# HeewoongNoh/DOSTransformer

Hardware: NVIDIA B200
Metric: train-step crystals/sec (fwd+bwd) (higher is better)
Workload: dtype bf16x3 operands, f32 accumulate

## Files before the change

### dostransformer_b200/_lib.py

```python
from __future__ import annotations

import ctypes as C
import os
from typing import Optional

import torch

_HERE = os.path.dirname(os.path.abspath(__file__))
LIB_PATH = os.environ.get("DOST_B200_LIB") or os.path.join(_HERE, "libdost_b200.so")

F32, F64 = 0, 1
ACT_NONE, ACT_RELU, ACT_LEAKY, ACT_PRELU = 0, 1, 2, 3
KC, MC = 0, 1
PREC_FMA, PREC_BF16X3, PREC_BF16 = 0, 1, 2
PRECISIONS = {"fp32": PREC_FMA, "bf16x3": PREC_BF16X3, "bf16": PREC_BF16}

_lib: Optional[C.CDLL] = None
ABI_VERSION = 15
DEVERR_MESSAGES = {1: "an index (edge_index / batch / system) is outside its table",
                   2: "a crystal has more atoms than the padding length given by the host (max_num_nodes)"}


class Seg(C.Structure):
    _fields_ = [("base", C.c_void_p), ("ld", C.c_longlong), ("idx", C.c_void_p), ("div", C.c_int),
# ... 36 lines not shown
        ("res_bstride", C.c_longlong),
        ("b_rowoff", C.c_void_p), ("c_rowoff", C.c_void_p), ("c_rowlim", C.c_void_p),
        ("colsum", C.c_void_p),
        ("out_gate", C.c_void_p), ("dact_gate", C.c_void_p), ("ld_gate", C.c_longlong),
    ]


_SIGNATURES = {
    "dost_abi_version": (C.c_int, []),
    "dost_last_error": (C.c_char_p, []),
    "dost_launch_count": (C.c_longlong, []),
    "dost_reset_launch_count": (None, []),
    "dost_device_errors_init": (C.c_int, []),
    "dost_device_errors": (C.c_uint, [C.c_int]),
    "dost_imax_scalar": (C.c_int, [C.c_void_p, C.c_int, C.c_void_p]),
    "dost_cast_i64_i32": (C.c_int, [C.c_void_p, C.c_void_p, C.c_longlong, C.c_void_p]),
    "dost_csr_workspace_bytes": (C.c_size_t, [C.c_longlong, C.c_longlong]),
    "dost_csr_build": (C.c_int, [C.c_void_p, C.c_longlong, C.c_longlong, C.c_void_p, C.c_void_p, C.c_void_p,
                                 C.c_void_p, C.c_size_t, C.c_void_p]),
    "dost_gemm_workspace_bytes": (C.c_size_t, [C.POINTER(Gemm)]),
    "dost_gemm": (C.c_int, [C.POINTER(Gemm), C.c_void_p, C.c_size_t, C.c_void_p]),
    "dost_gemm_bf16_workspace_bytes": (C.c_size_t, [C.POINTER(GemmBf16)]),
    "dost_gemm_bf16": (C.c_int, [C.POINTER(GemmBf16), C.c_void_p, C.c_size_t, C.c_void_p]),
    "dost_split_planes": (C.c_int, [C.c_void_p, C.c_longlong, C.c_longlong, C.c_int, C.c_void_p, C.c_void_p, C.c_longlong,
                                    C.c_void_p]),
    "dost_split_planes_multi": (C.c_int, [C.c_int, C.c_void_p, C.c_void_p, C.c_void_p, C.c_void_p, C.c_void_p, C.c_void_p,
                                          C.c_void_p, C.c_void_p]),
    "dost_split_planes_colsum_workspace_bytes": (C.c_size_t, [C.c_longlong, C.c_int, C.c_longlong]),
    "dost_split_planes_colsum": (C.c_int, [C.c_void_p, C.c_longlong, C.c_longlong, C.c_int, C.c_void_p, C.c_void_p, C.c_longlong,
                                           C.c_void_p, C.c_void_p, C.c_size_t, C.c_void_p]),
    "dost_ln_fwd_planes": (C.c_int, [C.c_void_p, C.c_longlong, C.c_void_p, C.c_void_p, C.c_void_p, C.c_void_p, C.c_longlong,
                                     C.c_void_p, C.c_void_p, C.c_void_p, C.c_void_p,
                                     C.c_void_p, C.c_void_p, C.c_longlong, C.c_void_p, C.c_longlong, C.c_int, C.c_void_p]),
    "dost_ln_bwd_planes_workspace_bytes": (C.c_size_t, [C.c_longlong, C.c_int]),
    "dost_ln_bwd_planes": (C.c_int, [C.c_void_p, C.c_longlong, C.c_void_p, C.c_longlong, C.c_void_p, C.c_void_p, C.c_void_p,
                                     C.c_void_p, C.c_void_p, C.c_longlong, C.c_void_p, C.c_void_p, C.c_void_p, C.c_longlong,
                                     C.c_void_p, C.c_void_p, C.c_void_p, C.c_void_p, C.c_longlong, C.c_int, C.c_void_p,
                                     C.c_size_t, C.c_void_p]),
    "dost_rowdot_fwd": (C.c_int, [C.c_void_p, C.c_longlong, C.c_void_p, C.c_void_p, C.c_void_p, C.c_longlong, C.c_int, C.c_void_p]),
    "dost_rowdot_bwd_workspace_bytes": (C.c_size_t, [C.c_longlong, C.c_int]),
    "dost_rowdot_bwd": (C.c_int, [C.c_void_p, C.c_void_p, C.c_longlong, C.c_void_p, C.c_void_p, C.c_void_p, C.c_longlong, C.c_int,
                                  C.c_void_p, C.c_size_t, C.c_void_p]),
    "dost_colsum_planes_workspace_bytes": (C.c_size_t, [C.c_longlong, C.c_int]),
    "dost_colsum_planes": (C.c_int, [C.c_void_p, C.c_void_p, C.c_longlong, C.c_longlong, C.c_int, C.c_void_p, C.c_void_p,
                                     C.c_size_t, C.c_void_p]),
    "dost_ln_fwd": (C.c_int, [C.c_int, C.c_void_p, C.c_longlong, C.c_void_p, C.c_void_p, C.c_void_p, C.c_void_p,
# ... 190 lines not shown
```

### dostransformer_b200/csrc/gemm_bf.cu

```cuda
#include <cuda.h>
#include <cuda_bf16.h>
#include <cstdlib>
#include "common.cuh"
#include "tc_ptx.cuh"

namespace dost {
namespace bf {

constexpr int BM = 128, BK = 64;
constexpr int kMaxStages = 6;
constexpr int kEpiBytes = 8 * 4096;
constexpr int kSmemBudget = 225 * 1024;

struct Maps {
  CUtensorMap a_hi[3], a_lo[3], b_hi, b_lo;
  CUtensorMap b_hi2, b_lo2;
  CUtensorMap c_out, c_hi, c_lo;
  CUtensorMap c_pre;
};

struct Params {
  int M, N, K;
  int a_nseg, a_kend[3];
  int a_mc, b_mc;
  int zmode, kchunk;
  long long c_bstride, res_bstride;
  const int* b_rowoff;
  const int* c_rowoff;
  const int* c_rowlim;
  int m_tiles, n_tiles, total_tiles;
  const float* bias;
  const float* rowbias; long long ld_rowbias; int rowbias_div;
  int act; float act_slope; const float* prelu_slope;
  float* out_pre; long long ld_pre;
  const __nv_bfloat16* dact_hi; long long ld_dact; float dact_slope;
  const float* residual; long long ld_res;
  float* out; long long ldc; int accumulate;
  __nv_bfloat16* out_hi; __nv_bfloat16* out_lo; long long ld_op;
  float* ws;
  float* colpart;
  unsigned int* out_gate;
  const unsigned int* dact_gate;
  long long ld_gate;
  int tma_epi;
};

// ... 115 lines not shown
                   : "memory");
      asm volatile("tcgen05.relinquish_alloc_permit.cta_group::1.sync.aligned;" ::: "memory");
    }
  }
  tc_fence_before();
  __syncthreads();
  if (CTA2) cluster_sync_all();
  tc_fence_after();
  const uint32_t tmem_base = tmem_base_s;
  const bool a_mc = p.a_mc != 0, b_mc = p.b_mc != 0;

  if (warp == kEpiWarps + 1) {
    if (lane == 0) {
      int stage = 0;
      uint32_t phase = 0;
      for (int tile = tile0; tile < p.total_tiles; tile += tile_step) {
        const TileInfo t = tile_info<BN, CTA2>(p, tile, rank);
        const int nb0 = t.n0 + rank * BNL;
        int seg = 0;
        for (int kt = 0; kt < t.nkt; ++kt) {
          const int k0 = t.kbeg + kt * BK;
          while (seg + 1 < p.a_nseg && k0 >= p.a_kend[seg]) ++seg;
          const int kseg = k0 - (seg == 0 ? 0 : p.a_kend[seg - 1]);
          mbar_wait(empty0 + 8 * stage, phase ^ 1);
          const uint32_t bar = CTA2 ? mapa_rank(full0 + 8 * stage, 0) : full0 + 8 * stage;
          if (!CTA2) mbar_expect_tx(bar, STAGE_BYTES);
          else if (rank == 0) mbar_expect_tx(full0 + 8 * stage, 2 * STAGE_BYTES);
          const uint32_t sA = smem_u32(smem + stage * STAGE_BYTES);
          const uint32_t sB = sA + (SPLIT ? 2 : 1) * A_BYTES;
          const int zb = (p.zmode == 1) ? t.z : 0;
          auto load = [&](uint32_t dst, const CUtensorMap* m, int c0, int c1, int c2) {
            if (CTA2) tma_load_3d_2cta(dst, m, c0, c1, c2, bar);
            else tma_load_3d(dst, m, c0, c1, c2, bar);
          };
          const int brow = p.b_rowoff ? __ldg(p.b_rowoff + t.z) : 0;
          const int zbb = p.b_rowoff ? 0 : zb;
          if (!a_mc) {
            load(sA, &maps.a_hi[seg], kseg, t.m0, zb);
            if (SPLIT) load(sA + A_BYTES, &maps.a_lo[seg], kseg, t.m0, zb);
          } else {
#pragma unroll
            for (int b = 0; b < BM / 64; ++b) {
              load(sA + b * 8192, &maps.a_hi[0], t.m0 + 64 * b, k0, zb);
              if (SPLIT) load(sA + A_BYTES + b * 8192, &maps.a_lo[0], t.m0 + 64 * b, k0, zb);
            }
          }
          if (!b_mc) {
            load(sB, CTA2 ? &maps.b_hi2 : &maps.b_hi, k0, nb0 + brow, zbb);
            if (SPLIT) load(sB + B_BYTES, CTA2 ? &maps.b_lo2 : &maps.b_lo, k0, nb0 + brow, zbb);
          } else {
#pragma unroll
            for (int b = 0; b < BNL / 64; ++b) {
              load(sB + b * 8192, &maps.b_hi, nb0 + 64 * b, k0 + brow, zbb);
              if (SPLIT) load(sB + B_BYTES + b * 8192, &maps.b_lo, nb0 + 64 * b, k0 + brow, zbb);
            }
          }
          if (++stage == NSTAGE) {
            stage = 0;
            phase ^= 1;
          }
        }
      }
    }
  } else if (warp == kEpiWarps) {
    const uint32_t idesc = make_idesc(CTA2 ? 2 * BM : BM, BN, a_mc, b_mc);
    const uint32_t a_kstep = a_mc ? (2048 >> 4) : (32 >> 4);
    const uint32_t b_kstep = b_mc ? (2048 >> 4) : (32 >> 4);
    int stage = 0;
    uint32_t phase = 0;
    uint32_t acc_phase[2] = {0, 0};
    int local = 0;
    for (int tile = tile0; tile < p.total_tiles && rank == 0; tile += tile_step, ++local) {
      const TileInfo t = tile_info<BN, CTA2>(p, tile, rank);
      const int buf = local & 1;
      mbar_wait(acce0 + 8 * buf, acc_phase[buf] ^ 1);
      tc_fence_after();
      const uint32_t tmem_d = tmem_base + buf * BN;
// ... 746 lines not shown
  attr[0].val.clusterDim.x = 2;
  attr[0].val.clusterDim.y = 1;
  attr[0].val.clusterDim.z = 1;
  cfg.attrs = attr;
  cfg.numAttrs = 1;
  cudaError_t e = cudaLaunchKernelEx(&cfg, kern, maps, p);
  if (e != cudaSuccess) {
    set_error("gemm_bf16: cluster launch failed: %s", cudaGetErrorString(e));
    return DOST_ERR_LAUNCH;
  }
  return check_launch("gemm_bf16 (CTA pairs)");
}

static bool use_cta_pairs(int M, int N) {
  static const int enabled = [] {
    const char* e = getenv("DOST_GEMM_2CTA");
    return (e && e[0] == '0') ? 0 : 1;
  }();
  return enabled && M > 128 && N > 128;
}

static inline bool al16(const void* ptr) { return (reinterpret_cast<uintptr_t>(ptr) & 15) == 0; }

static int run(const dost_gemm_bf16_t* h, void* workspace, size_t workspace_bytes, cudaStream_t st) {
  DOST_REQUIRE(h->M > 0 && h->N > 0 && h->K > 0, "gemm_bf16: bad shape M=%d N=%d K=%d", h->M, h->N, h->K);
  DOST_REQUIRE(h->precision == DOST_PREC_BF16X3 || h->precision == DOST_PREC_BF16, "gemm_bf16: precision must be bf16x3 or bf16");
  DOST_REQUIRE(h->N % 4 == 0, "gemm_bf16: N must be a multiple of 4 (got %d)", h->N);
  const bool split3 = h->precision == DOST_PREC_BF16X3;
  const bool a_mc = h->a_mode == DOST_MC, b_mc = h->b_mode == DOST_MC;
  const int nseg = a_mc ? 1 : h->a_nseg;
  DOST_REQUIRE(nseg >= 1 && nseg <= 3, "gemm_bf16: a_nseg must be 1..3");
  const int bn = h->N <= 64 ? 64 : (h->N <= 128 ? 128 : 256);
  const bool pairs = use_cta_pairs(h->M, h->N);
  const int batch = h->batch < 1 ? 1 : h->batch;
  DOST_REQUIRE(!(batch > 1 && h->split_k > 1), "gemm_bf16: batch and split_k are exclusive");
  DOST_REQUIRE(batch == 1 || (h->a_nseg <= 1 && !h->rowbias && !h->out_pre && !h->dact_hi && !h->out_hi),
               "gemm_bf16: batched problems support bias / activation / residual / fp32 stores only");
  DOST_REQUIRE(batch == 1 || (h->a_bstride % 8 == 0 && h->b_bstride % 8 == 0 && h->c_bstride % 4 == 0 && h->res_bstride % 4 == 0),
               "gemm_bf16: batch strides must keep 16-byte alignment");

  Maps maps;
  Params p;
  p.M = h->M; p.N = h->N; p.K = h->K;
  p.a_nseg = nseg;
  p.a_mc = a_mc; p.b_mc = b_mc;
  int kacc = 0;
  for (int s = 0; s < nseg; ++s) {
    const dost_planes_t& pl = h->a[s];
    DOST_REQUIRE(pl.hi && (!split3 || pl.lo), "gemm_bf16: A segment %d planes missing", s);
    DOST_REQUIRE(al16(pl.hi) && al16(pl.lo) && pl.ld % 8 == 0, "gemm_bf16: A segment %d planes must be 16-byte aligned, ld %% 8 == 0", s);
    const int width = a_mc ? h->K : pl.width;
    if (nseg > 1) DOST_REQUIRE(width % BK == 0, "gemm_bf16: concatenated A segments need widths %% 64 == 0 (got %d)", width);
    kacc += width;
    p.a_kend[s] = kacc;
    int rc;
    if (!a_mc) {
      const long long rows = batch > 1 ? h->M : pl.rows;
      rc = make_map(&maps.a_hi[s], pl.hi, width, rows, pl.ld, BM, batch, h->a_bstride);
      if (rc == DOST_OK && split3) rc = make_map(&maps.a_lo[s], pl.lo, width, rows, pl.ld, BM, batch, h->a_bstride);
    } else {
      rc = make_map(&maps.a_hi[s], pl.hi, h->M, h->K, pl.ld, 64, batch, h->a_bstride);
      if (rc == DOST_OK && split3) rc = make_map(&maps.a_lo[s], pl.lo, h->M, h->K, pl.ld, 64, batch, h->a_bstride);
    }
    if (rc != DOST_OK) return rc;
    if (!split3) maps.a_lo[s] = maps.a_hi[s];
  }
  for (int s = nseg; s < 3; ++s) {
    maps.a_hi[s] = maps.a_hi[0];
    maps.a_lo[s] = maps.a_lo[0];
    p.a_kend[s] = kacc;
  }
  DOST_REQUIRE(kacc == h->K, "gemm_bf16: A segment widths sum to %d, K=%d", kacc, h->K);
  {
    const dost_planes_t& pl = h->b;
    DOST_REQUIRE(pl.hi && (!split3 || pl.lo), "gemm_bf16: B planes missing");
    DOST_REQUIRE(al16(pl.hi) && al16(pl.lo) && pl.ld % 8 == 0, "gemm_bf16: B planes must be 16-byte aligned, ld %% 8 == 0");
    int rc;
    const bool ragged_b = h->b_rowoff != nullptr;
    if (ragged_b) {
      DOST_REQUIRE(pl.rows > 0, "gemm_bf16: ragged B needs the total number of stored rows");
      if (!b_mc) {
        rc = make_map(&maps.b_hi, pl.hi, h->K, pl.rows, pl.ld, bn);
        if (rc == DOST_OK && split3) rc = make_map(&maps.b_lo, pl.lo, h->K, pl.rows, pl.ld, bn);
        if (rc == DOST_OK && pairs) rc = make_map(&maps.b_hi2, pl.hi, h->K, pl.rows, pl.ld, 128);
        if (rc == DOST_OK && pairs && split3) rc = make_map(&maps.b_lo2, pl.lo, h->K, pl.rows, pl.ld, 128);
      } else {
        rc = make_map(&maps.b_hi, pl.hi, h->N, pl.rows, pl.ld, 64);
        if (rc == DOST_OK && split3) rc = make_map(&maps.b_lo, pl.lo, h->N, pl.rows, pl.ld, 64);
      }
    } else if (!b_mc) {
      const long long nrows = (pl.rows > 0 && pl.rows < h->N) ? pl.rows : h->N;
      rc = make_map(&maps.b_hi, pl.hi, h->K, nrows, pl.ld, bn, batch, h->b_bstride);
      if (rc == DOST_OK && split3) rc = make_map(&maps.b_lo, pl.lo, h->K, nrows, pl.ld, bn, batch, h->b_bstride);
      if (rc == DOST_OK && pairs) rc = make_map(&maps.b_hi2, pl.hi, h->K, nrows, pl.ld, 128, batch, h->b_bstride);
      if (rc == DOST_OK && pairs && split3) rc = make_map(&maps.b_lo2, pl.lo, h->K, nrows, pl.ld, 128, batch, h->b_bstride);
    } else {
      rc = make_map(&maps.b_hi, pl.hi, h->N, h->K, pl.ld, 64, batch, h->b_bstride);
      if (rc == DOST_OK && split3) rc = make_map(&maps.b_lo, pl.lo, h->N, h->K, pl.ld, 64, batch, h->b_bstride);
    }
    if (rc != DOST_OK) return rc;
    if (!split3) maps.b_lo = maps.b_hi;
    if (!pairs || b_mc) maps.b_hi2 = maps.b_hi;
    if (!pairs || b_mc || !split3) maps.b_lo2 = maps.b_hi2;
  }
  const int split = h->split_k < 1 ? 1 : h->split_k;
  p.zmode = split > 1 ? 2 : (batch > 1 ? 1 : 0);
  p.c_bstride = h->c_bstride;
  p.res_bstride = h->res_bstride;
  p.b_rowoff = h->b_rowoff;
  p.c_rowoff = h->c_rowoff;
  p.c_rowlim = h->c_rowlim;
  DOST_REQUIRE(!p.c_rowoff || p.c_rowlim, "gemm_bf16: ragged output needs both c_rowoff and c_rowlim");
  DOST_REQUIRE(split == 1 || !(p.b_rowoff || p.c_rowoff || p.c_rowlim), "gemm_bf16: ragged problems cannot be split along K");
  p.kchunk = 0;
  p.ws = nullptr;
  if (split > 1) {
    DOST_REQUIRE(!h->bias && !h->rowbias && h->act == DOST_ACT_NONE && !h->out_pre && !h->dact_hi && !h->residual && !h->out_hi,
                 "gemm_bf16: split_k supports only plain (accumulating) fp32 stores");
    const size_t need = sizeof(float) * (size_t)split * h->M * h->N;
    if (!workspace || workspace_bytes < need) {
      set_error("gemm_bf16: split_k workspace too small (%zu < %zu)", workspace_bytes, need);
      return DOST_ERR_WORKSPACE;
    }
    int kchunk = (h->K + split - 1) / split;
    p.kchunk = ((kchunk + BK - 1) / BK) * BK;
    p.ws = (float*)workspace;
// ... 21 lines not shown
  p.colpart = nullptr;
  const int nrb = (h->M + 31) / 32;
  if (h->colsum) {
    DOST_REQUIRE(split == 1 && batch == 1, "gemm_bf16: colsum needs a plain (single, un-split) problem");
    const size_t need = sizeof(float) * ((size_t)nrb + kMidRows) * h->N;
    if (!workspace || workspace_bytes < need) {
      set_error("gemm_bf16: colsum workspace too small (%zu < %zu)", workspace_bytes, need);
      return DOST_ERR_WORKSPACE;
    }
    p.colpart = (float*)workspace;
  }
  DOST_REQUIRE(h->out || h->out_hi, "gemm_bf16: no output");
  DOST_REQUIRE(!h->out || (al16(h->out) && h->ldc % 4 == 0), "gemm_bf16: out must be 16-byte aligned with ldc %% 4 == 0");
  DOST_REQUIRE(!h->bias || al16(h->bias), "gemm_bf16: bias must be 16-byte aligned");
  DOST_REQUIRE(!h->rowbias || (al16(h->rowbias) && h->ld_rowbias % 4 == 0), "gemm_bf16: rowbias alignment");
  DOST_REQUIRE(!h->out_pre || (al16(h->out_pre) && h->ld_pre % 4 == 0), "gemm_bf16: out_pre alignment");
  DOST_REQUIRE(!h->residual || (al16(h->residual) && h->ld_res % 4 == 0), "gemm_bf16: residual alignment");
  DOST_REQUIRE(!h->dact_hi || (((uintptr_t)h->dact_hi & 7) == 0 && h->ld_dact % 4 == 0), "gemm_bf16: dact plane alignment");
  DOST_REQUIRE(!h->out_hi || (((uintptr_t)h->out_hi & 7) == 0 && ((uintptr_t)h->out_lo & 7) == 0 && h->ld_op % 4 == 0),
               "gemm_bf16: output plane alignment");

  p.tma_epi = 0;
  bool ew16 = false;
  maps.c_out = maps.b_hi;
  maps.c_hi = maps.b_hi;
  maps.c_lo = maps.b_hi;
  maps.c_pre = maps.b_hi;
  if (tma_epi_enabled() && split == 1 && !(h->accumulate && h->out_hi) && !p.c_rowoff && !p.c_rowlim &&
      !(h->out_pre && !h->out) && (batch == 1 || !h->out_hi) && h->M >= 32 && h->N >= 32 && !(h->dact_hi && h->residual) &&
      (!h->dact_hi || (al16(h->dact_hi) && h->ld_dact % 8 == 0))) {
    int rc2 = DOST_OK;
    ew16 = pairs && epi16_enabled(h->colsum != nullptr);
    const int bc = ew16 ? 16 : 32;
    if (h->out) rc2 = make_out_map(&maps.c_out, h->out, true, bc, h->N, h->M, h->ldc, batch, h->c_bstride);
    if (rc2 == DOST_OK && h->out_pre) rc2 = make_out_map(&maps.c_pre, h->out_pre, true, bc, h->N, h->M, h->ld_pre);
    if (rc2 == DOST_OK && h->out_hi) {
      if (al16(h->out_hi) && al16(h->out_lo) && h->ld_op % 8 == 0) {
        rc2 = make_out_map(&maps.c_hi, h->out_hi, false, bc, h->N, h->M, h->ld_op);
        if (rc2 == DOST_OK && h->out_lo) rc2 = make_out_map(&maps.c_lo, h->out_lo, false, bc, h->N, h->M, h->ld_op);
      } else {
        rc2 = DOST_ERR_ARG;
      }
    }
    if (rc2 == DOST_OK) p.tma_epi = 1;
    else ew16 = false;
  }

  if ((h->out_gate || h->dact_gate) && !p.tma_epi) {
    set_error("gemm_bf16: activation gates are implemented by the TMA-store epilogue only (this launch is not eligible)");
    return DOST_ERR_UNSUPPORTED;
// ... 17 lines not shown
  }
  if (split > 1) {
    const long long total4 = (long long)h->M * h->N / 4;
    int blocks = (int)min64((total4 + 255) / 256, (long long)kNumSMs * 8);
    if (blocks < 1) blocks = 1;
    splitk_reduce_kernel<<<blocks, 256, 0, st>>>(p.ws, h->out, h->ldc, h->M, h->N, split, h->accumulate);
    rc = check_launch("gemm_bf16 split-k reduce");
  }
  return rc;
}

}
}

extern "C" size_t dost_gemm_bf16_workspace_bytes(const dost_gemm_bf16_t* g) {
  if (!g) return 0;
  if (g->colsum) return sizeof(float) * ((size_t)((g->M + 31) / 32) + dost::bf::kMidRows) * g->N;
  if (g->split_k <= 1) return 0;
  return sizeof(float) * (size_t)g->split_k * g->M * g->N;
}

extern "C" int dost_gemm_bf16(const dost_gemm_bf16_t* g, void* workspace, size_t workspace_bytes, dost_stream_t stream) {
  DOST_REQUIRE(g != nullptr, "gemm_bf16: null descriptor");
  return dost::bf::run(g, workspace, workspace_bytes, (cudaStream_t)stream);
}

extern "C" size_t dost_split_planes_colsum_workspace_bytes(long long rows, int cols, long long ldp) {
  return sizeof(float) * (size_t)dost::bf::split_colsum_chunks(rows, (int)ldp) * cols;
}

extern "C" int dost_split_planes_colsum(const float* x, long long ld, long long rows, int cols, void* hi, void* lo, long long ldp,
                                        float* colsum, void* workspace, size_t workspace_bytes, dost_stream_t stream) {
  DOST_REQUIRE(x && hi && colsum, "split_planes_colsum: null pointer");
  DOST_REQUIRE(rows > 0 && cols > 0 && ldp >= cols && ldp % 8 == 0, "split_planes_colsum: need rows > 0, ldp %% 8 == 0, ldp >= cols");
  DOST_REQUIRE(((uintptr_t)hi & 15) == 0 && ((uintptr_t)lo & 15) == 0, "split_planes_colsum: planes must be 16-byte aligned");
  const int nch = dost::bf::split_colsum_chunks(rows, (int)ldp);
  const size_t need = sizeof(float) * (size_t)nch * cols;
  if (!workspace || workspace_bytes < need) {
    dost::set_error("split_planes_colsum: workspace too small (%zu < %zu)", workspace_bytes, need);
    return DOST_ERR_WORKSPACE;
  }
  const int vec_ok = (((uintptr_t)x & 15) == 0 && ld % 4 == 0) ? 1 : 0;
  const long long rpc = (rows + nch - 1) / nch;
  dim3 grid((unsigned)((ldp / 8 + 31) / 32), nch);
  cudaStream_t st = (cudaStream_t)stream;
  dost::bf::split_planes_colsum_kernel<<<grid, 256, 0, st>>>(x, ld, rows, cols, (__nv_bfloat16*)hi, (__nv_bfloat16*)lo, (int)ldp, vec_ok,
                                                             rpc, (float*)workspace);
// ... 55 lines not shown
```

### dostransformer_b200/ops.py

```python
from __future__ import annotations

import ctypes as C
import math
from contextlib import nullcontext
import os
from dataclasses import dataclass, field
from typing import List, Optional, Sequence, Tuple

import torch

from . import _lib as L

NUM_SMS = 148

_PRECISION = L.PREC_FMA


def set_precision(name: str) -> None:
    global _PRECISION
    _PRECISION = L.PRECISIONS[name]


def get_precision() -> int:
    return _PRECISION
# ... 361 lines not shown
        cache[_planes_key(w)] = ((base._version, base.data_ptr(), _PLANES_GENERATION), Planes(hi, lo, w.shape[0], w.shape[1]))


def _planes_c(pl: Planes, width: int) -> L.PlanesC:
    c = L.PlanesC()
    c.hi = pl.hi.data_ptr()
    c.lo = pl.lo.data_ptr() if pl.lo is not None else None
    c.ld = pl.ld
    c.rows = pl.rows
    c.width = width
    return c


def gemm_planes(*, M: int, N: int, K: int, a: Sequence[Planes], a_mode: int, b: Planes, b_mode: int,
                out: Optional[torch.Tensor] = None, bias: Optional[torch.Tensor] = None,
                rowbias: Optional[torch.Tensor] = None, rowbias_div: int = 1, act: int = L.ACT_NONE, act_slope: float = 0.0,
                prelu_slope: Optional[torch.Tensor] = None, out_pre: Optional[torch.Tensor] = None,
                dact: Optional[Planes] = None, dact_slope: float = 0.0, residual: Optional[torch.Tensor] = None,
                accumulate: bool = False, split_k: int = 1, out_planes: Optional[Planes] = None,
                ldc: Optional[int] = None, prec: Optional[int] = None, batch: int = 1, a_bstride: int = 0, b_bstride: int = 0,
                c_bstride: int = 0, res_bstride: int = 0, ld_res: Optional[int] = None, b_rows: Optional[int] = None,
                b_rowoff: Optional[torch.Tensor] = None, c_rowoff: Optional[torch.Tensor] = None,
                c_rowlim: Optional[torch.Tensor] = None, colsum_out: Optional[torch.Tensor] = None,
                out_gate: Optional[torch.Tensor] = None, dact_gate: Optional[torch.Tensor] = None) -> None:
    g = L.GemmBf16()
    g.M, g.N, g.K = M, N, K
    g.a_mode, g.a_nseg = a_mode, len(a)
    for i, pl in enumerate(a):
        g.a[i] = _planes_c(pl, pl.cols if a_mode == L.KC else K)
    g.b_mode = b_mode
    g.b = _planes_c(b, 0)
    g.b.rows = b_rows if b_rows is not None else 0
    g.bias = bias.data_ptr() if bias is not None else None
    if rowbias is not None:
        g.rowbias, g.ld_rowbias, g.rowbias_div = rowbias.data_ptr(), _ld(rowbias), rowbias_div
    g.act, g.act_slope = act, act_slope
    g.prelu_slope = prelu_slope.data_ptr() if prelu_slope is not None else None
    if out_pre is not None:
        g.out_pre, g.ld_pre = out_pre.data_ptr(), _ld(out_pre)
    if dact is not None:
        g.dact_hi, g.ld_dact, g.dact_slope = dact.hi.data_ptr(), dact.ld, dact_slope
    if residual is not None:
        g.residual, g.ld_res = residual.data_ptr(), (ld_res if ld_res is not None else _ld(residual))
    if out is not None:
        g.out = out.data_ptr()
        g.ldc = ldc if ldc is not None else _ld(out)
    g.accumulate = 1 if accumulate else 0
    g.batch, g.a_bstride, g.b_bstride, g.c_bstride, g.res_bstride = batch, a_bstride, b_bstride, c_bstride, res_bstride
    g.b_rowoff = b_rowoff.data_ptr() if b_rowoff is not None else None
    g.c_rowoff = c_rowoff.data_ptr() if c_rowoff is not None else None
    g.c_rowlim = c_rowlim.data_ptr() if c_rowlim is not None else None
    if out_planes is not None:
        g.out_hi = out_planes.hi.data_ptr()
        g.out_lo = out_planes.lo.data_ptr() if out_planes.lo is not None else None
        g.ld_op = out_planes.ld
    g.split_k = split_k
    g.precision = _PRECISION if prec is None else prec
    g.colsum = colsum_out.data_ptr() if colsum_out is not None else None
    if out_gate is not None:
        g.out_gate, g.ld_gate = out_gate.data_ptr(), out_gate.stride(0)
    if dact_gate is not None:
        g.dact_gate, g.ld_gate, g.dact_slope = dact_gate.data_ptr(), dact_gate.stride(0), dact_slope
    lib = L.lib()
    ws, nb = None, 0
    if split_k > 1 or colsum_out is not None:
        nb = lib.dost_gemm_bf16_workspace_bytes(C.byref(g))
        ws = _ws(nb, b.hi.device)
    L.check(lib.dost_gemm_bf16(C.byref(g), L.p(ws), nb, L.stream()), "gemm_bf16")


def gate_bits_ok(M: int, N: int) -> bool:
    return M >= 32 and N % 32 == 0 and os.environ.get("DOST_GEMM_TMA_EPI", "1") != "0" and not L.switch("DOST_NO_FFN_GATE")


def tc_active(t: torch.Tensor) -> bool:
    return _PRECISION != L.PREC_FMA and t.dtype == torch.float32


def _with_lo() -> bool:
    return _PRECISION != L.PREC_BF16


def ln_fwd_planes(x2d: torch.Tensor, gamma, beta, slope=None, *, want_y: bool = False, want_planes: bool = True,
                  gather_add=None):
    M, W = x2d.shape
    ga = ia = gb = ib = None
    ldg = 0
    if gather_add is not None:
        ga, ia, gb, ib = gather_add
        ldg = _ld(ga)
        assert _ld(gb) == ldg
# ... 869 lines not shown
            dop = _grad_planes(d_out, S * T, H)
            d_out = d_out.contiguous()
            dP = torch.empty(S * T, npad, dtype=torch.float32, device=dev)
            gemm_planes(M=T, N=npad, K=H, a=[dop], a_mode=L.KC, b=kvp, b_mode=L.KC, b_rows=N + B, out=dP, batch=S,
                        a_bstride=T * dop.ld, c_bstride=T * npad, b_rowoff=ptr_ext)
            dsp = empty_planes(S * T, npad, dev, _with_lo())
            if ctx.fused and ctx.drop_p > 0:
                scores = torch.empty(S * T, npad, dtype=torch.float32, device=dev)
                gemm_planes(M=T, N=npad, K=H, a=[qp], a_mode=L.KC, b=kvp, b_mode=L.KC, b_rows=N + B, out=scores, batch=S,
                            a_bstride=T * qp.ld, c_bstride=T * npad, b_rowoff=ptr_ext)
            if ctx.fused and ctx.drop_p == 0:
                _ds_from_planes(pp, dP, S * T, npad, float(H) ** -0.5, dsp)
            else:
                L.check(lib.dost_xattn_softmax_bwd_dseed(L.p(scores), L.p(lse), L.p(dP), L.p(g.ptr), L.p(g.nmax), S * T, B, T, npad,
                                                         float(H) ** -0.5, L.p(dsp.hi), L.p(dsp.lo), dsp.ld, ctx.drop_p, ctx.seed,
                                                         L.p(ctx.seed_offset), L.stream()), "xattn_softmax_bwd")
            dq = torch.empty(S, T, H, dtype=torch.float32, device=dev)
            gemm_planes(M=T, N=H, K=npad, a=[dsp], a_mode=L.KC, b=kvp, b_mode=L.MC, b_rows=N + B, out=dq.view(S * T, H), batch=S,
                        a_bstride=T * dsp.ld, c_bstride=T * H, b_rowoff=ptr_ext)
            dkv = torch.empty(N, H, dtype=torch.float32, device=dev)
            dbrows = torch.empty(B, H, dtype=torch.float32, device=dev)
            if not L.switch("DOST_NO_XATTN_PADDED_DK"):
                dpad = torch.empty(S * npad, H, dtype=torch.float32, device=dev)
                gemm_planes(M=npad, N=H, K=T, a=[dsp], a_mode=L.MC, b=qp, b_mode=L.MC, out=dpad, batch=S, a_bstride=T * dsp.ld,
                            b_bstride=T * qp.ld, c_bstride=npad * H)
                gemm_planes(M=npad, N=H, K=T, a=[pp], a_mode=L.MC, b=dop, b_mode=L.MC, out=dpad, accumulate=True, batch=S,
                            a_bstride=T * pp.ld, b_bstride=T * dop.ld, c_bstride=npad * H)
                L.check(lib.dost_xattn_kv_pad_split(L.p(dpad), npad, reps, L.p(g.batch), L.p(g.ptr), N, B, H, L.p(dkv), L.p(dbrows),
                                                    L.stream()), "xattn_kv_pad_split")
                dph = colsum(dbrows)
                d_q = colsum(dq.view(S, T * H)).view(T, H) if ctx.bcast_q else dq
                d_resid = colsum(d_out.view(S, T * H)).view(T, H) if ctx.bcast_r else d_out
                return d_q, dkv, dph, d_resid, None, None, None, None, None, None
            dext = torch.empty(N + B, H, dtype=torch.float32, device=dev)
            p1, n1 = g.ragged(1)
            for rep in range(reps):
                r0, r1 = rep * B * T, (rep + 1) * B * T
                gemm_planes(M=npad, N=H, K=T, a=[_rows(dsp, r0, r1)], a_mode=L.MC, b=_rows(qp, r0, r1), b_mode=L.MC, out=dext,
                            accumulate=rep > 0, batch=B, a_bstride=T * dsp.ld, b_bstride=T * qp.ld, c_rowoff=p1, c_rowlim=n1)
                gemm_planes(M=npad, N=H, K=T, a=[_rows(pp, r0, r1)], a_mode=L.MC, b=_rows(dop, r0, r1), b_mode=L.MC, out=dext,
                            accumulate=True, batch=B, a_bstride=T * pp.ld, b_bstride=T * dop.ld, c_rowoff=p1, c_rowlim=n1)
            L.check(lib.dost_xattn_kv_ext_split(L.p(dext), L.p(g.batch), L.p(g.ptr), N, B, H, L.p(dkv), L.p(dbrows), L.stream()),
                    "xattn_kv_ext_split")
            dph = colsum(dbrows)
            d_q = colsum(dq.view(S, T * H)).view(T, H) if ctx.bcast_q else dq
            d_resid = colsum(d_out.view(S, T * H)).view(T, H) if ctx.bcast_r else d_out
        return d_q, dkv, dph, d_resid, None, None, None, None, None, None


def _rows(pl: Planes, r0: int, r1: int) -> Planes:
# ... 108 lines not shown
    qp, kp = Planes(qh, ql, S * Lq, H), Planes(kh, kl, S * Lk, H)
    pdp = Planes(ph, pl_, S * Lq, Lk)
    dop = _grad_planes(d_out, S * Lq, H)
    d_out = d_out.contiguous()
    dpd = torch.empty(S, Lq, Lp, dtype=torch.float32, device=dev)
    gemm_planes(M=Lq, N=Lp, K=H, a=[dop], a_mode=L.KC, b=kp, b_mode=L.KC, b_rows=Lk, out=dpd.view(S * Lq, Lp), batch=S,
                a_bstride=Lq * dop.ld, b_bstride=Lk * kp.ld, c_bstride=Lq * Lp)
    dsp = empty_planes(S * Lq, Lk, dev, _with_lo())
    if ctx.fused and ctx.drop_p > 0:
        prob = torch.empty(S, Lq, Lp, dtype=torch.float32, device=dev)
        gemm_planes(M=Lq, N=Lp, K=H, a=[qp], a_mode=L.KC, b=kp, b_mode=L.KC, b_rows=Lk, out=prob.view(S * Lq, Lp), batch=S,
                    a_bstride=Lq * qp.ld, b_bstride=Lk * kp.ld, c_bstride=Lq * Lp)
        L.check(L.lib().dost_softmax_fwd(L.F32, L.p(prob), L.p(prob), None, S * Lq, Lk, Lp, scale, 0.0, 0, L.stream()), "softmax_fwd")
    if ctx.fused and ctx.drop_p == 0:
        _ds_from_planes(pdp, dpd.view(S * Lq, Lp), S * Lq, Lk, scale, dsp)
    else:
        L.check(L.lib().dost_softmax_bwd_planes_dseed(L.p(prob), L.p(dpd), None, S * Lq, Lk, Lp, scale, ctx.drop_p, ctx.seed,
                                                      L.p(ctx.seed_offset), L.p(dsp.hi), L.p(dsp.lo), dsp.ld, L.stream()),
                "softmax_bwd_planes")
    dq = torch.empty(S, Lq, H, dtype=torch.float32, device=dev)
    gemm_planes(M=Lq, N=H, K=Lk, a=[dsp], a_mode=L.KC, b=kp, b_mode=L.MC, out=dq.view(S * Lq, H), batch=S,
                a_bstride=Lq * dsp.ld, b_bstride=Lk * kp.ld, c_bstride=Lq * H)
    dk = torch.empty(S, Lk, H, dtype=torch.float32, device=dev)
    gemm_planes(M=Lk, N=H, K=Lq, a=[dsp], a_mode=L.MC, b=qp, b_mode=L.MC, out=dk.view(S * Lk, H), batch=S,
                a_bstride=Lq * dsp.ld, b_bstride=Lq * qp.ld, c_bstride=Lk * H)
    gemm_planes(M=Lk, N=H, K=Lq, a=[pdp], a_mode=L.MC, b=dop, b_mode=L.MC, out=dk.view(S * Lk, H), accumulate=True, batch=S,
                a_bstride=Lq * pdp.ld, b_bstride=Lq * dop.ld, c_bstride=Lk * H)
    return dq, dk, d_out, None, None, None


_SelfAttention._backward_planes = staticmethod(_self_attention_backward_planes)


def _cols(pl: Planes, cols: int) -> Planes:
    return Planes(pl.hi, pl.lo, pl.rows, cols)


def _planes3(t: torch.Tensor) -> Optional[Planes]:
    pl = getattr(t, "_dost_planes", None)
    if pl is not None and t.dim() == 3 and pl.rows == t.shape[0] * t.shape[1] and pl.cols == t.shape[2] and \
            (pl.lo is not None) == _with_lo():
        return pl
    return None


def self_attention(q, k, resid, drop_p: float = 0.0, seed: int = 0, seed_offset=None):
    _check_seed_offset(seed_offset)
    out = _SelfAttention.apply(q, k, resid, drop_p, seed, seed_offset)
    if tc_active(q) and q.shape[-1] % 8 == 0:
        out._dost_attn_out = True
# ... 91 lines not shown
```

### include/dost.h

```cpp
#ifndef DOST_H_
#define DOST_H_

#include <stddef.h>
#include <stdint.h>

#ifdef __cplusplus
extern "C" {
#endif

#define DOST_ABI_VERSION 15

enum { DOST_F32 = 0, DOST_F64 = 1 };
enum { DOST_OK = 0, DOST_ERR_ARG = -1, DOST_ERR_LAUNCH = -2, DOST_ERR_WORKSPACE = -3, DOST_ERR_UNSUPPORTED = -4 };
enum { DOST_ACT_NONE = 0, DOST_ACT_RELU = 1, DOST_ACT_LEAKY = 2, DOST_ACT_PRELU = 3 };
enum { DOST_PREC_FMA = 0, DOST_PREC_BF16X3 = 1 , DOST_PREC_BF16 = 2 };
enum { DOST_KC = 0 , DOST_MC = 1  };

typedef void* dost_stream_t;

int dost_abi_version(void);
const char* dost_last_error(void);
long long dost_launch_count(void);
void dost_reset_launch_count(void);

// ... 60 lines not shown
  const float* bias;
  const float* rowbias; long long ld_rowbias; int rowbias_div;
  int act; float act_slope; const float* prelu_slope;
  float* out_pre; long long ld_pre;
  const void* dact_hi; long long ld_dact; float dact_slope;
  const float* residual; long long ld_res;
  float* out; long long ldc; int accumulate;
  void* out_hi; void* out_lo; long long ld_op;
  int split_k;
  int precision;
  int batch;
  long long a_bstride, b_bstride, c_bstride, res_bstride;
  const int32_t* b_rowoff;
  const int32_t* c_rowoff;
  const int32_t* c_rowlim;
  float* colsum;
  uint32_t* out_gate;
  const uint32_t* dact_gate;
  long long ld_gate;
} dost_gemm_bf16_t;

size_t dost_gemm_bf16_workspace_bytes(const dost_gemm_bf16_t* g);
int dost_gemm_bf16(const dost_gemm_bf16_t* g, void* workspace, size_t workspace_bytes, dost_stream_t stream);
int dost_split_planes_multi(int ntensors, const float* const* x, const long long* ld, const long long* rows, const int* cols,
                            void* const* hi, void* const* lo, const long long* ldp, dost_stream_t stream);
int dost_split_planes(const float* x, long long ld, long long rows, int cols, void* hi, void* lo, long long ldp,
                      dost_stream_t stream);
size_t dost_split_planes_colsum_workspace_bytes(long long rows, int cols, long long ldp);
int dost_split_planes_colsum(const float* x, long long ld, long long rows, int cols, void* hi, void* lo, long long ldp,
                             float* colsum, void* workspace, size_t workspace_bytes, dost_stream_t stream);

int dost_ln_fwd_planes(float* x, long long ldx, const float* ga, const int32_t* ia, const float* gb, const int32_t* ib,
                       long long ldg, const float* gamma, const float* beta, const float* prelu_slope, float* y,
                       void* hi, void* lo, long long ldp, float* stats, long long M, int W, dost_stream_t stream);
size_t dost_ln_bwd_planes_workspace_bytes(long long M, int W);
int dost_ln_bwd_planes(const float* dy, long long ld_dy, const float* x, long long ldx, const float* stats,
                       const float* gamma, const float* beta, const float* prelu_slope, const float* dres,
                       long long ld_dres, float* dx, void* dx_hi, void* dx_lo, long long ldp, float* dgamma,
                       float* dbeta, float* dslope, float* dxsum, long long M, int W, void* workspace,
                       size_t workspace_bytes, dost_stream_t stream);
int dost_rowdot_fwd(const float* x, long long ldx, const float* w, const float* bias, float* out, long long M, int K,
                    dost_stream_t stream);
size_t dost_rowdot_bwd_workspace_bytes(long long M, int K);
int dost_rowdot_bwd(const float* dout, const float* x, long long ldx, const float* w, float* dx, float* dwb, long long M, int K,
                    void* workspace, size_t workspace_bytes, dost_stream_t stream);
size_t dost_colsum_planes_workspace_bytes(long long M, int W);
// ... 146 lines not shown
```

Baseline: 21360.

## Fuse two accumulating attention-backward GEMMs into one two-product GEMM launch

```diff
diff --git a/dostransformer_b200/_lib.py b/dostransformer_b200/_lib.py
--- a/dostransformer_b200/_lib.py
+++ b/dostransformer_b200/_lib.py
@@ -82,6 +82,7 @@
     "dost_gemm": (C.c_int, [C.POINTER(Gemm), C.c_void_p, C.c_size_t, C.c_void_p]),
     "dost_gemm_bf16_workspace_bytes": (C.c_size_t, [C.POINTER(GemmBf16)]),
     "dost_gemm_bf16": (C.c_int, [C.POINTER(GemmBf16), C.c_void_p, C.c_size_t, C.c_void_p]),
+    "dost_gemm_bf16_two_products": (C.c_int, [C.POINTER(GemmBf16), C.POINTER(PlanesC), C.c_void_p, C.c_size_t, C.c_void_p]),
     "dost_split_planes": (C.c_int, [C.c_void_p, C.c_longlong, C.c_longlong, C.c_int, C.c_void_p, C.c_void_p, C.c_longlong,
                                     C.c_void_p]),
     "dost_split_planes_multi": (C.c_int, [C.c_int, C.c_void_p, C.c_void_p, C.c_void_p, C.c_void_p, C.c_void_p, C.c_void_p,
diff --git a/dostransformer_b200/csrc/gemm_bf.cu b/dostransformer_b200/csrc/gemm_bf.cu
--- a/dostransformer_b200/csrc/gemm_bf.cu
+++ b/dostransformer_b200/csrc/gemm_bf.cu
@@ -13,8 +13,9 @@
 constexpr int kSmemBudget = 225 * 1024;
 
 struct Maps {
-  CUtensorMap a_hi[3], a_lo[3], b_hi, b_lo;
-  CUtensorMap b_hi2, b_lo2;
+  CUtensorMap a_hi[3], a_lo[3];
+  CUtensorMap b_hi[2], b_lo[2];
+  CUtensorMap b_hi2[2], b_lo2[2];
   CUtensorMap c_out, c_hi, c_lo;
   CUtensorMap c_pre;
 };
@@ -22,6 +23,7 @@
 struct Params {
   int M, N, K;
   int a_nseg, a_kend[3];
+  int b_seg;
   int a_mc, b_mc;
   int zmode, kchunk;
   long long c_bstride, res_bstride;
@@ -183,6 +185,8 @@
           const int k0 = t.kbeg + kt * BK;
           while (seg + 1 < p.a_nseg && k0 >= p.a_kend[seg]) ++seg;
           const int kseg = k0 - (seg == 0 ? 0 : p.a_kend[seg - 1]);
+          const int bs = p.b_seg ? seg : 0;
+          const int kb = p.b_seg ? kseg : k0;
           mbar_wait(empty0 + 8 * stage, phase ^ 1);
           const uint32_t bar = CTA2 ? mapa_rank(full0 + 8 * stage, 0) : full0 + 8 * stage;
           if (!CTA2) mbar_expect_tx(bar, STAGE_BYTES);
@@ -202,18 +206,18 @@
           } else {
 #pragma unroll
             for (int b = 0; b < BM / 64; ++b) {
-              load(sA + b * 8192, &maps.a_hi[0], t.m0 + 64 * b, k0, zb);
-              if (SPLIT) load(sA + A_BYTES + b * 8192, &maps.a_lo[0], t.m0 + 64 * b, k0, zb);
+              load(sA + b * 8192, &maps.a_hi[seg], t.m0 + 64 * b, kseg, zb);
+              if (SPLIT) load(sA + A_BYTES + b * 8192, &maps.a_lo[seg], t.m0 + 64 * b, kseg, zb);
             }
           }
           if (!b_mc) {
-            load(sB, CTA2 ? &maps.b_hi2 : &maps.b_hi, k0, nb0 + brow, zbb);
-            if (SPLIT) load(sB + B_BYTES, CTA2 ? &maps.b_lo2 : &maps.b_lo, k0, nb0 + brow, zbb);
+            load(sB, CTA2 ? &maps.b_hi2[bs] : &maps.b_hi[bs], kb, nb0 + brow, zbb);
+            if (SPLIT) load(sB + B_BYTES, CTA2 ? &maps.b_lo2[bs] : &maps.b_lo[bs], kb, nb0 + brow, zbb);
           } else {
 #pragma unroll
             for (int b = 0; b < BNL / 64; ++b) {
-              load(sB + b * 8192, &maps.b_hi, nb0 + 64 * b, k0 + brow, zbb);
-              if (SPLIT) load(sB + B_BYTES + b * 8192, &maps.b_lo, nb0 + 64 * b, k0 + brow, zbb);
+              load(sB + b * 8192, &maps.b_hi[bs], nb0 + 64 * b, kb + brow, zbb);
+              if (SPLIT) load(sB + B_BYTES + b * 8192, &maps.b_lo[bs], nb0 + 64 * b, kb + brow, zbb);
             }
           }
           if (++stage == NSTAGE) {
@@ -1006,20 +1010,28 @@
 
 static inline bool al16(const void* ptr) { return (reinterpret_cast<uintptr_t>(ptr) & 15) == 0; }
 
-static int run(const dost_gemm_bf16_t* h, void* workspace, size_t workspace_bytes, cudaStream_t st) {
+static int run(const dost_gemm_bf16_t* h, const dost_planes_t* b_seg1, void* workspace, size_t workspace_bytes, cudaStream_t st) {
   DOST_REQUIRE(h->M > 0 && h->N > 0 && h->K > 0, "gemm_bf16: bad shape M=%d N=%d K=%d", h->M, h->N, h->K);
   DOST_REQUIRE(h->precision == DOST_PREC_BF16X3 || h->precision == DOST_PREC_BF16, "gemm_bf16: precision must be bf16x3 or bf16");
   DOST_REQUIRE(h->N % 4 == 0, "gemm_bf16: N must be a multiple of 4 (got %d)", h->N);
   const bool split3 = h->precision == DOST_PREC_BF16X3;
   const bool a_mc = h->a_mode == DOST_MC, b_mc = h->b_mode == DOST_MC;
-  const int nseg = a_mc ? 1 : h->a_nseg;
+  const bool bseg = b_seg1 != nullptr;
+  const int nseg = (a_mc && !bseg) ? 1 : h->a_nseg;
   DOST_REQUIRE(nseg >= 1 && nseg <= 3, "gemm_bf16: a_nseg must be 1..3");
+  DOST_REQUIRE(!bseg || nseg == 2, "gemm_bf16: a second B needs a_nseg == 2");
   const int bn = h->N <= 64 ? 64 : (h->N <= 128 ? 128 : 256);
   const bool pairs = use_cta_pairs(h->M, h->N);
   const int batch = h->batch < 1 ? 1 : h->batch;
   DOST_REQUIRE(!(batch > 1 && h->split_k > 1), "gemm_bf16: batch and split_k are exclusive");
-  DOST_REQUIRE(batch == 1 || (h->a_nseg <= 1 && !h->rowbias && !h->out_pre && !h->dact_hi && !h->out_hi),
-               "gemm_bf16: batched problems support bias / activation / residual / fp32 stores only");
+  DOST_REQUIRE(batch == 1 || ((h->a_nseg <= 1 || bseg) && !h->rowbias && !h->out_pre && !h->dact_hi && !h->out_hi),
+               "gemm_bf16: batched problems support bias / activation / residual / fp32 stores / two products only");
+  DOST_REQUIRE(!bseg || batch == 1 || (h->a[1].ld == h->a[0].ld && b_seg1->ld == h->b.ld),
+               "gemm_bf16: batched two-product problems need equal plane pitches of both pairs");
+  if (bseg && (h->split_k > 1 || h->b_rowoff)) {
+    set_error("gemm_bf16: two-product problems cannot be split along K or use a ragged B");
+    return DOST_ERR_UNSUPPORTED;
+  }
   DOST_REQUIRE(batch == 1 || (h->a_bstride % 8 == 0 && h->b_bstride % 8 == 0 && h->c_bstride % 4 == 0 && h->res_bstride % 4 == 0),
                "gemm_bf16: batch strides must keep 16-byte alignment");
 
@@ -1027,15 +1039,18 @@
   Params p;
   p.M = h->M; p.N = h->N; p.K = h->K;
   p.a_nseg = nseg;
+  p.b_seg = bseg ? 1 : 0;
   p.a_mc = a_mc; p.b_mc = b_mc;
-  int kacc = 0;
+  int kacc = 0, ksum = 0;
   for (int s = 0; s < nseg; ++s) {
     const dost_planes_t& pl = h->a[s];
     DOST_REQUIRE(pl.hi && (!split3 || pl.lo), "gemm_bf16: A segment %d planes missing", s);
     DOST_REQUIRE(al16(pl.hi) && al16(pl.lo) && pl.ld % 8 == 0, "gemm_bf16: A segment %d planes must be 16-byte aligned, ld %% 8 == 0", s);
-    const int width = a_mc ? h->K : pl.width;
-    if (nseg > 1) DOST_REQUIRE(width % BK == 0, "gemm_bf16: concatenated A segments need widths %% 64 == 0 (got %d)", width);
-    kacc += width;
+    const int width = (a_mc && !bseg) ? h->K : pl.width;
+    DOST_REQUIRE(width > 0, "gemm_bf16: A segment %d is empty", s);
+    if (nseg > 1 && !bseg) DOST_REQUIRE(width % BK == 0, "gemm_bf16: concatenated A segments need widths %% 64 == 0 (got %d)", width);
+    ksum += width;
+    kacc += (bseg && s + 1 < nseg) ? (width + BK - 1) / BK * BK : width;
     p.a_kend[s] = kacc;
     int rc;
     if (!a_mc) {
@@ -1043,8 +1058,8 @@
       rc = make_map(&maps.a_hi[s], pl.hi, width, rows, pl.ld, BM, batch, h->a_bstride);
       if (rc == DOST_OK && split3) rc = make_map(&maps.a_lo[s], pl.lo, width, rows, pl.ld, BM, batch, h->a_bstride);
     } else {
-      rc = make_map(&maps.a_hi[s], pl.hi, h->M, h->K, pl.ld, 64, batch, h->a_bstride);
-      if (rc == DOST_OK && split3) rc = make_map(&maps.a_lo[s], pl.lo, h->M, h->K, pl.ld, 64, batch, h->a_bstride);
+      rc = make_map(&maps.a_hi[s], pl.hi, h->M, width, pl.ld, 64, batch, h->a_bstride);
+      if (rc == DOST_OK && split3) rc = make_map(&maps.a_lo[s], pl.lo, h->M, width, pl.ld, 64, batch, h->a_bstride);
     }
     if (rc != DOST_OK) return rc;
     if (!split3) maps.a_lo[s] = maps.a_hi[s];
@@ -1054,9 +1069,11 @@
     maps.a_lo[s] = maps.a_lo[0];
     p.a_kend[s] = kacc;
   }
-  DOST_REQUIRE(kacc == h->K, "gemm_bf16: A segment widths sum to %d, K=%d", kacc, h->K);
-  {
-    const dost_planes_t& pl = h->b;
+  DOST_REQUIRE(ksum == h->K, "gemm_bf16: A segment widths sum to %d, K=%d", ksum, h->K);
+  p.K = kacc;
+  for (int s = 0; s < (bseg ? 2 : 1); ++s) {
+    const dost_planes_t& pl = s == 0 ? h->b : *b_seg1;
+    const int kb = bseg ? h->a[s].width : h->K;
     DOST_REQUIRE(pl.hi && (!split3 || pl.lo), "gemm_bf16: B planes missing");
     DOST_REQUIRE(al16(pl.hi) && al16(pl.lo) && pl.ld % 8 == 0, "gemm_bf16: B planes must be 16-byte aligned, ld %% 8 == 0");
     int rc;
@@ -1064,28 +1081,32 @@
     if (ragged_b) {
       DOST_REQUIRE(pl.rows > 0, "gemm_bf16: ragged B needs the total number of stored rows");
       if (!b_mc) {
-        rc = make_map(&maps.b_hi, pl.hi, h->K, pl.rows, pl.ld, bn);
-        if (rc == DOST_OK && split3) rc = make_map(&maps.b_lo, pl.lo, h->K, pl.rows, pl.ld, bn);
-        if (rc == DOST_OK && pairs) rc = make_map(&maps.b_hi2, pl.hi, h->K, pl.rows, pl.ld, 128);
-        if (rc == DOST_OK && pairs && split3) rc = make_map(&maps.b_lo2, pl.lo, h->K, pl.rows, pl.ld, 128);
+        rc = make_map(&maps.b_hi[s], pl.hi, kb, pl.rows, pl.ld, bn);
+        if (rc == DOST_OK && split3) rc = make_map(&maps.b_lo[s], pl.lo, kb, pl.rows, pl.ld, bn);
+        if (rc == DOST_OK && pairs) rc = make_map(&maps.b_hi2[s], pl.hi, kb, pl.rows, pl.ld, 128);
+        if (rc == DOST_OK && pairs && split3) rc = make_map(&maps.b_lo2[s], pl.lo, kb, pl.rows, pl.ld, 128);
       } else {
-        rc = make_map(&maps.b_hi, pl.hi, h->N, pl.rows, pl.ld, 64);
-        if (rc == DOST_OK && split3) rc = make_map(&maps.b_lo, pl.lo, h->N, pl.rows, pl.ld, 64);
+        rc = make_map(&maps.b_hi[s], pl.hi, h->N, pl.rows, pl.ld, 64);
+        if (rc == DOST_OK && split3) rc = make_map(&maps.b_lo[s], pl.lo, h->N, pl.rows, pl.ld, 64);
       }
     } else if (!b_mc) {
       const long long nrows = (pl.rows > 0 && pl.rows < h->N) ? pl.rows : h->N;
-      rc = make_map(&maps.b_hi, pl.hi, h->K, nrows, pl.ld, bn, batch, h->b_bstride);
-      if (rc == DOST_OK && split3) rc = make_map(&maps.b_lo, pl.lo, h->K, nrows, pl.ld, bn, batch, h->b_bstride);
-      if (rc == DOST_OK && pairs) rc = make_map(&maps.b_hi2, pl.hi, h->K, nrows, pl.ld, 128, batch, h->b_bstride);
-      if (rc == DOST_OK && pairs && split3) rc = make_map(&maps.b_lo2, pl.lo, h->K, nrows, pl.ld, 128, batch, h->b_bstride);
+      rc = make_map(&maps.b_hi[s], pl.hi, kb, nrows, pl.ld, bn, batch, h->b_bstride);
+      if (rc == DOST_OK && split3) rc = make_map(&maps.b_lo[s], pl.lo, kb, nrows, pl.ld, bn, batch, h->b_bstride);
+      if (rc == DOST_OK && pairs) rc = make_map(&maps.b_hi2[s], pl.hi, kb, nrows, pl.ld, 128, batch, h->b_bstride);
+      if (rc == DOST_OK && pairs && split3) rc = make_map(&maps.b_lo2[s], pl.lo, kb, nrows, pl.ld, 128, batch, h->b_bstride);
     } else {
-      rc = make_map(&maps.b_hi, pl.hi, h->N, h->K, pl.ld, 64, batch, h->b_bstride);
-      if (rc == DOST_OK && split3) rc = make_map(&maps.b_lo, pl.lo, h->N, h->K, pl.ld, 64, batch, h->b_bstride);
+      rc = make_map(&maps.b_hi[s], pl.hi, h->N, kb, pl.ld, 64, batch, h->b_bstride);
+      if (rc == DOST_OK && split3) rc = make_map(&maps.b_lo[s], pl.lo, h->N, kb, pl.ld, 64, batch, h->b_bstride);
     }
     if (rc != DOST_OK) return rc;
-    if (!split3) maps.b_lo = maps.b_hi;
-    if (!pairs || b_mc) maps.b_hi2 = maps.b_hi;
-    if (!pairs || b_mc || !split3) maps.b_lo2 = maps.b_hi2;
+    if (!split3) maps.b_lo[s] = maps.b_hi[s];
+    if (!pairs || b_mc) maps.b_hi2[s] = maps.b_hi[s];
+    if (!pairs || b_mc || !split3) maps.b_lo2[s] = maps.b_hi2[s];
+  }
+  if (!bseg) {
+    maps.b_hi[1] = maps.b_hi[0]; maps.b_lo[1] = maps.b_lo[0];
+    maps.b_hi2[1] = maps.b_hi2[0]; maps.b_lo2[1] = maps.b_lo2[0];
   }
   const int split = h->split_k < 1 ? 1 : h->split_k;
   p.zmode = split > 1 ? 2 : (batch > 1 ? 1 : 0);
@@ -1153,10 +1174,10 @@
 
   p.tma_epi = 0;
   bool ew16 = false;
-  maps.c_out = maps.b_hi;
-  maps.c_hi = maps.b_hi;
-  maps.c_lo = maps.b_hi;
-  maps.c_pre = maps.b_hi;
+  maps.c_out = maps.b_hi[0];
+  maps.c_hi = maps.b_hi[0];
+  maps.c_lo = maps.b_hi[0];
+  maps.c_pre = maps.b_hi[0];
   if (tma_epi_enabled() && split == 1 && !(h->accumulate && h->out_hi) && !p.c_rowoff && !p.c_rowlim &&
       !(h->out_pre && !h->out) && (batch == 1 || !h->out_hi) && h->M >= 32 && h->N >= 32 && !(h->dact_hi && h->residual) &&
       (!h->dact_hi || (al16(h->dact_hi) && h->ld_dact % 8 == 0))) {
@@ -1220,7 +1241,13 @@
 
 extern "C" int dost_gemm_bf16(const dost_gemm_bf16_t* g, void* workspace, size_t workspace_bytes, dost_stream_t stream) {
   DOST_REQUIRE(g != nullptr, "gemm_bf16: null descriptor");
-  return dost::bf::run(g, workspace, workspace_bytes, (cudaStream_t)stream);
+  return dost::bf::run(g, nullptr, workspace, workspace_bytes, (cudaStream_t)stream);
+}
+
+extern "C" int dost_gemm_bf16_two_products(const dost_gemm_bf16_t* g, const dost_planes_t* b_seg1, void* workspace,
+                                           size_t workspace_bytes, dost_stream_t stream) {
+  DOST_REQUIRE(g != nullptr && b_seg1 != nullptr && b_seg1->hi != nullptr, "gemm_bf16_two_products: null descriptor or second B");
+  return dost::bf::run(g, b_seg1, workspace, workspace_bytes, (cudaStream_t)stream);
 }
 
 extern "C" size_t dost_split_planes_colsum_workspace_bytes(long long rows, int cols, long long ldp) {
diff --git a/dostransformer_b200/ops.py b/dostransformer_b200/ops.py
--- a/dostransformer_b200/ops.py
+++ b/dostransformer_b200/ops.py
@@ -407,12 +407,15 @@
                 c_bstride: int = 0, res_bstride: int = 0, ld_res: Optional[int] = None, b_rows: Optional[int] = None,
                 b_rowoff: Optional[torch.Tensor] = None, c_rowoff: Optional[torch.Tensor] = None,
                 c_rowlim: Optional[torch.Tensor] = None, colsum_out: Optional[torch.Tensor] = None,
-                out_gate: Optional[torch.Tensor] = None, dact_gate: Optional[torch.Tensor] = None) -> None:
+                out_gate: Optional[torch.Tensor] = None, dact_gate: Optional[torch.Tensor] = None,
+                b2: Optional[Planes] = None) -> None:
     g = L.GemmBf16()
     g.M, g.N, g.K = M, N, K
     g.a_mode, g.a_nseg = a_mode, len(a)
     for i, pl in enumerate(a):
         g.a[i] = _planes_c(pl, pl.cols if a_mode == L.KC else K)
+    if b2 is not None:
+        g.K = 2 * K
     g.b_mode = b_mode
     g.b = _planes_c(b, 0)
     g.b.rows = b_rows if b_rows is not None else 0
@@ -451,7 +454,11 @@
     if split_k > 1 or colsum_out is not None:
         nb = lib.dost_gemm_bf16_workspace_bytes(C.byref(g))
         ws = _ws(nb, b.hi.device)
-    L.check(lib.dost_gemm_bf16(C.byref(g), L.p(ws), nb, L.stream()), "gemm_bf16")
+    if b2 is not None:
+        L.check(lib.dost_gemm_bf16_two_products(C.byref(g), C.byref(_planes_c(b2, 0)), L.p(ws), nb, L.stream()),
+                "gemm_bf16_two_products")
+    else:
+        L.check(lib.dost_gemm_bf16(C.byref(g), L.p(ws), nb, L.stream()), "gemm_bf16")
 
 
 def gate_bits_ok(M: int, N: int) -> bool:
@@ -1367,10 +1374,8 @@
             dbrows = torch.empty(B, H, dtype=torch.float32, device=dev)
             if not L.switch("DOST_NO_XATTN_PADDED_DK"):
                 dpad = torch.empty(S * npad, H, dtype=torch.float32, device=dev)
-                gemm_planes(M=npad, N=H, K=T, a=[dsp], a_mode=L.MC, b=qp, b_mode=L.MC, out=dpad, batch=S, a_bstride=T * dsp.ld,
-                            b_bstride=T * qp.ld, c_bstride=npad * H)
-                gemm_planes(M=npad, N=H, K=T, a=[pp], a_mode=L.MC, b=dop, b_mode=L.MC, out=dpad, accumulate=True, batch=S,
-                            a_bstride=T * pp.ld, b_bstride=T * dop.ld, c_bstride=npad * H)
+                gemm_planes(M=npad, N=H, K=T, a=[dsp, pp], a_mode=L.MC, b=qp, b2=dop, b_mode=L.MC, out=dpad, batch=S,
+                            a_bstride=T * dsp.ld, b_bstride=T * qp.ld, c_bstride=npad * H)
                 L.check(lib.dost_xattn_kv_pad_split(L.p(dpad), npad, reps, L.p(g.batch), L.p(g.ptr), N, B, H, L.p(dkv), L.p(dbrows),
                                                     L.stream()), "xattn_kv_pad_split")
                 dph = colsum(dbrows)
@@ -1525,10 +1530,8 @@
     gemm_planes(M=Lq, N=H, K=Lk, a=[dsp], a_mode=L.KC, b=kp, b_mode=L.MC, out=dq.view(S * Lq, H), batch=S,
                 a_bstride=Lq * dsp.ld, b_bstride=Lk * kp.ld, c_bstride=Lq * H)
     dk = torch.empty(S, Lk, H, dtype=torch.float32, device=dev)
-    gemm_planes(M=Lk, N=H, K=Lq, a=[dsp], a_mode=L.MC, b=qp, b_mode=L.MC, out=dk.view(S * Lk, H), batch=S,
+    gemm_planes(M=Lk, N=H, K=Lq, a=[dsp, pdp], a_mode=L.MC, b=qp, b2=dop, b_mode=L.MC, out=dk.view(S * Lk, H), batch=S,
                 a_bstride=Lq * dsp.ld, b_bstride=Lq * qp.ld, c_bstride=Lk * H)
-    gemm_planes(M=Lk, N=H, K=Lq, a=[pdp], a_mode=L.MC, b=dop, b_mode=L.MC, out=dk.view(S * Lk, H), accumulate=True, batch=S,
-                a_bstride=Lq * pdp.ld, b_bstride=Lq * dop.ld, c_bstride=Lk * H)
     return dq, dk, d_out, None, None, None
 
 
diff --git a/include/dost.h b/include/dost.h
--- a/include/dost.h
+++ b/include/dost.h
@@ -106,6 +106,8 @@
 
 size_t dost_gemm_bf16_workspace_bytes(const dost_gemm_bf16_t* g);
 int dost_gemm_bf16(const dost_gemm_bf16_t* g, void* workspace, size_t workspace_bytes, dost_stream_t stream);
+int dost_gemm_bf16_two_products(const dost_gemm_bf16_t* g, const dost_planes_t* b_seg1, void* workspace,
+                                size_t workspace_bytes, dost_stream_t stream);
 int dost_split_planes_multi(int ntensors, const float* const* x, const long long* ld, const long long* rows, const int* cols,
                             void* const* hi, void* const* lo, const long long* ldp, dost_stream_t stream);
 int dost_split_planes(const float* x, long long ld, long long rows, int cols, void* hi, void* lo, long long ldp,
```

After: 21510 (median of 6 runs). No clear change (+0.7%).
